# marekrams/tnac4o

Measured on AMD Instinct MI355X. Metric: PEPS-contraction ms/sweep, chimera L=2048 chi=64 (boundary-MPS sweep _setup_rhoT), lower is better.
Workload: dtype f64; 1 GPU; chimera L=2048 (Nx=Ny=16, Nc=8), synthetic couplings seed 20260004, beta=3, chi=64; one sweep = 16 rows of MPO absorb + compress_mps; one step = the sweeps of the 4 lattice rotations of one instance; parallelism=1 GPU: 4 lattice rotations of one instance interleaved on 4 HIP streams, mode=sweep

## Files before the change

include/tnpeps.h:

```cpp
#ifndef TNPEPS_H
#define TNPEPS_H
#include <stdint.h>

#ifdef __cplusplus
extern "C" {
#endif

int tn_version(void);
int tn_build_id(char* buf, int n);
int tn_stream_create_masked(const uint32_t* mask_host, int nwords, void** stream_out);
int tn_stream_destroy(void* stream);
int tn_last_error(char* buf, int n);

int tn_gemm(int64_t M, int64_t N, int64_t K, double alpha, const double* A, int64_t rsa, int64_t csa,
            const double* B, int64_t rsb, int64_t csb, double beta, double* C, int64_t rsc, int64_t csc,
            int64_t batch, int64_t bsa, int64_t bsb, int64_t bsc, void* ws, int64_t ws_bytes, void* stream);
int64_t tn_gemm_ws_bytes(int64_t M, int64_t N, int64_t K, int64_t batch);

int tn_absorb(const double* A, const double* W, double* out, int64_t Dl, int64_t pold, int64_t Dr, int64_t ba,
              int64_t po, int64_t bb, int64_t pi, int hconj, int64_t batch, int64_t bsA, int64_t bsW, int64_t bsOut,
              void* stream);

int tn_qr(double* A, int64_t rs, int64_t cs, int64_t m, int64_t n, double* Q, int64_t qrs, int64_t qcs, double* R,
          int64_t rrs, int64_t rcs, int nb, double rank_tol, int64_t* keff_host, void* ws, int64_t ws_bytes, void* stream);
int64_t tn_qr_ws_bytes(int64_t m, int64_t n, int nb);
int64_t tn_panel_orth_ws_bytes(int64_t nrows, int b);
int tn_panel_orth(const double* X, int64_t rs, int64_t cs, int64_t nrows, int b, double* Y, int64_t yrs, int64_t ycs, int method,
                  int* state9_host, double* dev_host, void* ws, int64_t ws_bytes, void* stream);
int tn_panel_stats(uint64_t* out16_host, int reset);
int tn_panel_stats_stream(uint64_t* out16_host, int reset, void* stream);
int tn_smallqr_stats(uint64_t* out4_host, int reset, void* stream);
int tn_fused_timeouts(int* count_host, void* stream);
int tn_qr_batched(double* A, int64_t rs, int64_t cs, int64_t m, int64_t n, double* Q, int64_t qrs, int64_t qcs, double* R,
                  int64_t rrs, int64_t rcs, int nb, double rank_tol, int64_t* keff_host, int64_t batch, int64_t bsA, int64_t bsQ,
                  int64_t bsR, void* ws, int64_t ws_bytes, void* stream, void* const* side_streams, int nside);

int tn_svd_trunc(const double* C, int64_t crs, int64_t ccs, int64_t k, int64_t n, int64_t Dmax, double tol, double* U,
                 int64_t urs, int64_t ucs, double* S, double* Vt, int64_t vrs, int64_t vcs, int64_t* keep_host,
                 double* discarded_host, int* sweeps_host, int* info_host, void* ws, int64_t ws_bytes, void* stream);
int tn_svdvals(const double* C, int64_t crs, int64_t ccs, int64_t k, int64_t n, double* S_host, int* sweeps_host,
               int* info_host, void* ws, int64_t ws_bytes, void* stream);
int64_t tn_svd_ws_bytes(int64_t k, int64_t n, int vectors);
int tn_svdvals_async(const double* C, int64_t crs, int64_t ccs, int64_t k, int64_t n, double* out66_dev, void* stream);
int tn_svdvals_small_batched(const int64_t* desc_dev, int64_t batch, const int64_t* desc_host, double* out66_dev, void* stream);
int tn_svd_trunc_batched(const double* C, int64_t crs, int64_t ccs, int64_t k, int64_t n, int64_t Dmax, double tol, double* U,
                         int64_t urs, int64_t ucs, double* S, double* Vt, int64_t vrs, int64_t vcs, int64_t* keep_host,
                         double* discarded_host, int* sweeps_host, int* info_host, int64_t batch, int64_t bsC, int64_t bsU,
                         int64_t bsS, int64_t bsV, void* ws, int64_t ws_bytes, void* stream);
int tn_svdvals_batched(const double* C, int64_t crs, int64_t ccs, int64_t k, int64_t n, double* S_host, int* sweeps_host,
                       int* info_host, int64_t batch, int64_t bsC, void* ws, int64_t ws_bytes, void* stream);

int tn_nfactor(const double* x, int64_t n, double* out2, void* slot8, void* stream);
int tn_normalize_pow2(double* x, int64_t n, double* out2, void* scratch, int64_t scratch_bytes, void* stream);
int tn_scale_by(double* x, int64_t n, const double* scalar_dev, void* stream);
int tn_scale_phys(double* A, int64_t Dl, int64_t p, int64_t Dr, const double* diag, int inv, void* stream);

int tn_peps_factor(const double* Es, const double* E1, const double* E4, const double* Xu, const double* Xl, const double* Xr,
                   const double* Xd, const int32_t* dmap, const int32_t* rmap, int64_t q, int64_t nl, int64_t nu, double* F,
                   void* stream);
int tn_mpo_from_factor(const double* F, const int32_t* dmap, const int32_t* rmap, int64_t q, int64_t nl, int64_t nu, int64_t pd,
                       int64_t br, double* W, void* stream);
int tn_mpo_from_factor_ops(const double* F, const int32_t* dmap, const int32_t* rmap, const double* O, int64_t nop, int64_t q, int64_t nl,
                           int64_t nu, int64_t pd, int64_t br, double* Wops, void* stream);

int tn_calc_pn(const double* T1, const double* RR, const double* F, const int32_t* dmap, const int32_t* rmap,
               const int32_t* pref, const int32_t* suf, const int32_t* lidx, const int32_t* uidx, int64_t nb,
               int64_t q, int64_t nl, int64_t nu, int64_t p, int64_t Dr, int64_t br, double* P, double* minP,
               const double* parent_log2p, double* log2p_out, void* stream);
int tn_sample_pn(const double* T1, const double* RR, const double* F, const int32_t* dmap, const int32_t* rmap, const int32_t* pref,
                 const int32_t* suf, const int32_t* lidx, const int32_t* uidx, const int32_t* perm, const int64_t* starts, int64_t ng,
// ... 124 lines not shown
```

tnac4o_amd/_lib.py:

```python
import ctypes as C
import os
import subprocess

HERE = os.path.dirname(os.path.abspath(__file__))
LIB_PATH = os.path.join(HERE, 'libtnpeps.so')
CSRC = os.path.join(HERE, 'csrc')
SOURCES = ['api.hip', 'gemm_f64.hip', 'rank_update.hip', 'small.hip', 'qr.hip', 'svd.hip', 'absorb.hip', 'misc.hip', 'beam.hip', 'prof.hip', 'cholqr.hip', 'smallqr.hip', 'fused.hip', 'peps.hip', 'env.hip', 'batch.hip', 'site.hip', 'chain.hip', 'beamsearch.hip', 'marginal.hip', 'sampler.hip', 'overlap.hip']

_i64, _f64, _int, _ptr = C.c_int64, C.c_double, C.c_int, C.c_void_p

SIGNATURES = {
    'tn_version': (_int, []),
    'tn_last_error': (_int, [C.c_char_p, _int]),
    'tn_build_id': (_int, [C.c_char_p, _int]),
    'tn_stream_create_masked': (_int, [C.POINTER(C.c_uint32), _int, C.POINTER(_ptr)]),
    'tn_stream_destroy': (_int, [_ptr]),
    'tn_gemm': (_int, [_i64, _i64, _i64, _f64, _ptr, _i64, _i64, _ptr, _i64, _i64, _f64, _ptr, _i64, _i64,
                       _i64, _i64, _i64, _i64, _ptr, _i64, _ptr]),
    'tn_gemm_ws_bytes': (_i64, [_i64, _i64, _i64, _i64]),
    'tn_absorb': (_int, [_ptr, _ptr, _ptr, _i64, _i64, _i64, _i64, _i64, _i64, _i64, _int, _i64, _i64, _i64, _i64, _ptr]),
    'tn_qr': (_int, [_ptr, _i64, _i64, _i64, _i64, _ptr, _i64, _i64, _ptr, _i64, _i64, _int, _f64, C.POINTER(_i64), _ptr, _i64,
              _ptr]),
    'tn_qr_ws_bytes': (_i64, [_i64, _i64, _int]),
    'tn_panel_orth_ws_bytes': (_i64, [_i64, _int]),
    'tn_panel_orth': (_int, [_ptr, _i64, _i64, _i64, _int, _ptr, _i64, _i64, _int, C.POINTER(_int), C.POINTER(_f64), _ptr, _i64, _ptr]),
    'tn_panel_stats': (_int, [C.POINTER(C.c_uint64), _int]),
    'tn_panel_stats_stream': (_int, [C.POINTER(C.c_uint64), _int, _ptr]),
    'tn_smallqr_stats': (_int, [C.POINTER(C.c_uint64), _int, _ptr]),
    'tn_fused_timeouts': (_int, [C.POINTER(_int), _ptr]),
    'tn_qr_batched': (_int, [_ptr, _i64, _i64, _i64, _i64, _ptr, _i64, _i64, _ptr, _i64, _i64, _int, _f64, C.POINTER(_i64), _i64, _i64, _i64,
                      _i64, _ptr, _i64, _ptr, C.POINTER(_ptr), _int]),
    'tn_svd_trunc': (_int, [_ptr, _i64, _i64, _i64, _i64, _i64, _f64, _ptr, _i64, _i64, _ptr, _ptr, _i64, _i64,
                            C.POINTER(_i64), C.POINTER(_f64), C.POINTER(_int), C.POINTER(_int), _ptr, _i64, _ptr]),
    'tn_svdvals': (_int, [_ptr, _i64, _i64, _i64, _i64, C.POINTER(_f64), C.POINTER(_int), C.POINTER(_int), _ptr, _i64,
                          _ptr]),
    'tn_svd_ws_bytes': (_i64, [_i64, _i64, _int]),
    'tn_svdvals_async': (_int, [_ptr, _i64, _i64, _i64, _i64, _ptr, _ptr]),
    'tn_svdvals_small_batched': (_int, [_ptr, _i64, _ptr, _ptr, _ptr]),
    'tn_svd_trunc_batched': (_int, [_ptr, _i64, _i64, _i64, _i64, _i64, _f64, _ptr, _i64, _i64, _ptr, _ptr, _i64, _i64, C.POINTER(_i64),
                             C.POINTER(_f64), C.POINTER(_int), C.POINTER(_int), _i64, _i64, _i64, _i64, _i64, _ptr, _i64, _ptr]),
    'tn_svdvals_batched': (_int, [_ptr, _i64, _i64, _i64, _i64, C.POINTER(_f64), C.POINTER(_int), C.POINTER(_int), _i64, _i64, _ptr, _i64,
                           _ptr]),
    'tn_nfactor': (_int, [_ptr, _i64, _ptr, _ptr, _ptr]),
    'tn_scale_by': (_int, [_ptr, _i64, _ptr, _ptr]),
    'tn_normalize_pow2': (_int, [_ptr, _i64, _ptr, _ptr, _i64, _ptr]),
    'tn_scale_phys': (_int, [_ptr, _i64, _i64, _i64, _ptr, _int, _ptr]),
    'tn_calc_pn': (_int, [_ptr] * 9 + [_i64] * 7 + [_ptr, _ptr, _ptr, _ptr, _ptr]),
    'tn_sample_pn': (_int, [_ptr] * 11 + [_i64, _ptr] + [_i64] * 6 + [_ptr, _ptr, _ptr, _ptr]),
    'tn_score_pn': (_int, [_ptr] * 11 + [_i64, _ptr] + [_i64] * 8 + [_ptr, _ptr, _ptr, _ptr, _ptr]),
    'tn_merge_groups': (_int, [_ptr] * 5 + [_i64, _f64, _ptr, _ptr, _ptr, _ptr]),
    'tn_mpo_from_factor_ops': (_int, [_ptr] * 4 + [_i64] * 6 + [_ptr, _ptr]),
    'tn_nfactor_batched': (_int, [_ptr, _i64, _i64, _ptr]),
    'tn_env_rr_batched': (_int, [_ptr] * 5 + [_i64] * 7 + [_ptr, _ptr]),
    'tn_env_rl_batched': (_int, [_ptr] * 3 + [_i64] * 3 + [_ptr, _ptr]),
    'tn_balance': (_int, [_ptr, _i64, _i64, _i64, _f64, _ptr, _ptr, _ptr]),
    'tn_peps_factor': (_int, [_ptr] * 9 + [_i64] * 3 + [_ptr, _ptr]),
    'tn_mpo_from_factor': (_int, [_ptr] * 3 + [_i64] * 5 + [_ptr, _ptr]),
    'tn_site_qr_ws_bytes': (_i64, [_int, _i64, _i64, _i64, _i64, _int]),
    'tn_site_qr': (_int, [_int, _ptr, _i64, _i64, _i64, _ptr, _i64, _ptr, _ptr, _f64, C.POINTER(_i64), _ptr, C.POINTER(_int), C.POINTER(_f64),
                   _int, C.POINTER(_i64), _ptr, _i64, _ptr]),
    'tn_gram_weights': (_int, [_ptr, _i64, _f64, _ptr, _ptr, _ptr]),
    'tn_rows_norm2': (_int, [_ptr, _i64, _i64, _ptr, _ptr]),
    'tn_gather_scale_rows': (_int, [_ptr, _i64, _i64, _ptr, _ptr, _ptr, _int, _ptr]),
    'tn_bond_deflate': (_int, [_int, _ptr, _i64, _i64, _ptr, _i64, _ptr, _ptr, C.POINTER(_i64), C.POINTER(_f64), _ptr, _i64, _ptr]),
    'tn_rar_ws_bytes': (_i64, [_i64] * 5),
    'tn_rar': (_int, [_ptr, _ptr, _ptr] + [_i64] * 5 + [_ptr, _ptr, _i64, _ptr]),
    'tn_env_mix_ws_bytes': (_i64, [_int] + [_i64] * 5),
    'tn_env_mix': (_int, [_int, _ptr, _ptr, _ptr] + [_i64] * 5 + [_ptr, _ptr, _i64, _ptr]),
    'tn_apply_truncation_ws_bytes': (_i64, [_i64] * 5),
    'tn_apply_truncation': (_int, [_ptr, _i64, _i64, _ptr, _i64, _i64, _i64, _ptr, _i64, _i64, _ptr, _i64, _i64, _ptr, _ptr, _ptr, _ptr, _ptr,
                            _i64, _ptr]),
    'tn_compress_mps_arena_bytes': (_i64, [_i64, C.POINTER(_i64), C.POINTER(_i64), _i64]),
# ... 67 lines not shown
    src_hash = source_hash()

    def one(s):
        src = os.path.join(CSRC, s)
        h = hh.copy()
        h.update(open(src, 'rb').read())
        extra = []
        if s == 'api.hip':
            extra = ['-DTN_SRC_HASH="%s"' % src_hash]
            h.update(src_hash.encode())
        obj = os.path.join(objdir, '%s.%s.o' % (s[:-4], h.hexdigest()[:16]))
        if not os.path.exists(obj):
            for old in os.listdir(objdir):
                if old.startswith(s[:-4] + '.') and old.endswith('.o'):
                    os.unlink(os.path.join(objdir, old))
            import tempfile
            fd, tmp = tempfile.mkstemp(prefix=s[:-4] + '.', suffix='.o.part', dir=objdir)
            os.close(fd)
            cmd = [hipcc] + flags + extra + ['-c', src, '-o', tmp]
            if verbose:
                print(' '.join(cmd), flush=True)
            try:
                subprocess.run(cmd, check=True)
                os.replace(tmp, obj)
            finally:
                if os.path.exists(tmp):
                    os.unlink(tmp)
        return obj

    with ThreadPoolExecutor(max_workers=int(os.environ.get('TN_BUILD_JOBS', '6'))) as ex:
        objs = list(ex.map(one, SOURCES))
    cmd = [hipcc, '--offload-arch=gfx950', '-shared', '-fPIC', '-Wl,--no-undefined'] + os.environ.get('TN_EXTRA_HIPCC_FLAGS', '').split() + ['-o', LIB_PATH] + objs
    if verbose:
        print(' '.join(cmd), flush=True)
    subprocess.run(cmd, check=True)
    return LIB_PATH


def _stale(L):
    buf = C.create_string_buffer(64)
    L.tn_build_id.restype, L.tn_build_id.argtypes = _int, [C.c_char_p, _int]
    L.tn_build_id(buf, 64)
    return buf.value.decode() != source_hash()


SHORT_CALLS = ('tn_gemm', 'tn_gemm_ws_bytes', 'tn_qr_ws_bytes', 'tn_svd_ws_bytes', 'tn_absorb', 'tn_nfactor', 'tn_scale_by',
               'tn_normalize_pow2', 'tn_scale_phys', 'tn_calc_pn', 'tn_sample_pn', 'tn_score_pn', 'tn_nfactor_batched', 'tn_env_rr_batched', 'tn_env_rl_batched',
               'tn_balance', 'tn_merge_groups', 'tn_svdvals_async', 'tn_rar', 'tn_rar_ws_bytes', 'tn_env_mix', 'tn_env_mix_ws_bytes',
               'tn_apply_truncation', 'tn_apply_truncation_ws_bytes', 'tn_site_qr_ws_bytes', 'tn_gram_weights', 'tn_argsort_desc', 'tn_weighted_sum', 'tn_rows_norm2', 'tn_gather_scale_rows', 'tn_peps_factor', 'tn_mpo_from_factor', 'tn_env3', 'tn_env3_ws_bytes',
               'tn_cluster_marginal', 'tn_cluster_marginal_ws_bytes', 'tn_cluster_bond_marginal', 'tn_cluster_bond_marginal_ws_bytes',
               'tn_mpo_from_factor_ops', 'tn_env3_stack', 'tn_env3_stack_ws_bytes', 'tn_stack_cell_law', 'tn_stack_cell_law_ws_bytes',
               'tn_last_error')
_lib = None
ABI_VERSION = 17


def lib():
    global _lib
    if _lib is None:
        if not os.path.exists(LIB_PATH):
            raise RuntimeError('libtnpeps.so not found at %s: run `python -c "import __graft_entry__ as g; g.build()"` '
                               '(the HIP library is the only backend; there is no CPU fallback)' % LIB_PATH)
        L = C.CDLL(LIB_PATH)
        L.tn_version.restype = _int
        if not hasattr(L, 'tn_build_id') or (_stale(L) and not os.environ.get('TN_ALLOW_STALE_LIB')):
            raise RuntimeError('libtnpeps.so was built from other sources than csrc/*.hip + include/tnpeps.h in this tree: '
                               'rebuild it with `python -c "import __graft_entry__ as g; g.build()"` -- a stale library can '
                               'disagree with the ctypes signatures declared here')
        if L.tn_version() != ABI_VERSION:
            raise RuntimeError('libtnpeps.so implements C-ABI version %d, this package binds version %d: rebuild the library'
                               % (L.tn_version(), ABI_VERSION))
        if os.environ.get('TN_PYDLL', '1') != '0':
            P = C.PyDLL(LIB_PATH)
            for name in SHORT_CALLS:
                setattr(L, name, getattr(P, name))
            L._pydll = P
        for name, (res, args) in SIGNATURES.items():
            fn = getattr(L, name)
            fn.restype, fn.argtypes = res, args
        _lib = L
    return _lib


class TnError(RuntimeError):
    pass


def check(rc):
    if rc != 0:
        buf = C.create_string_buffer(512)
        lib().tn_last_error(buf, 512)
        raise TnError('libtnpeps error %d: %s' % (rc, buf.value.decode(errors='replace')))
```

tnac4o_amd/csrc/api.hip:

```cpp
#include <stdarg.h>

#include "../../include/tnpeps.h"
#include "common.h"

namespace tn {

static thread_local char g_err[512] = "";

void set_error(const char* fmt, ...) {
    va_list ap;
    va_start(ap, fmt);
    vsnprintf(g_err, sizeof(g_err), fmt, ap);
    va_end(ap);
}
const char* get_error() { return g_err; }

}

using namespace tn;
#define ST ((hipStream_t)stream)

extern "C" {

int tn_version(void) { return 17; }

#ifndef TN_SRC_HASH
#define TN_SRC_HASH "unknown"
#endif
int tn_build_id(char* buf, int n) {
    const char* e = TN_SRC_HASH;
    const int len = (int)strlen(e);
    if (buf && n > 0) {
        const int c = len < n - 1 ? len : n - 1;
        memcpy(buf, e, c);
        buf[c] = 0;
    }
    return len;
}

void tn_profile_enable(unsigned mask) { prof_set_mask(mask); }
void tn_profile_reset(void) { prof_reset(); }
void tn_profile_sample(unsigned every) { prof_set_sample(every); }
int tn_profile_get(int family, uint64_t* calls_host, double* ms_host, double* flops_host, double* bytes_host) {
    TN_CHECK_ARG(family >= 0 && family < PROF_NFAM, "unknown kernel family");
    TN_CHECK_ARG(calls_host && ms_host && flops_host && bytes_host, "null output");
    prof_get(-1, family, calls_host, ms_host, flops_host, bytes_host);
    return 0;
}
int tn_profile_get_phase(int phase, int family, uint64_t* calls_host, double* ms_host, double* flops_host, double* bytes_host) {
    TN_CHECK_ARG(phase >= -1 && phase < PH_N, "unknown phase");
    TN_CHECK_ARG(family >= 0 && family < PROF_NFAM, "unknown kernel family");
    TN_CHECK_ARG(calls_host && ms_host && flops_host && bytes_host, "null output");
    prof_get(phase, family, calls_host, ms_host, flops_host, bytes_host);
    return 0;
}

int tn_stream_create_masked(const uint32_t* mask_host, int nwords, void** stream_out) {
    TN_CHECK_ARG(mask_host && nwords >= 1 && stream_out, "bad arguments");
    hipStream_t st = nullptr;
    const hipError_t e = hipExtStreamCreateWithCUMask(&st, (uint32_t)nwords, mask_host);
    if (e != hipSuccess) return hip_fail(e, "hipExtStreamCreateWithCUMask");
    fused_forms_disable(st);
    *stream_out = (void*)st;
    return 0;
}
int tn_stream_destroy(void* stream) {
    fused_stream_released((hipStream_t)stream);
    const hipError_t e = hipStreamDestroy((hipStream_t)stream);
    return e == hipSuccess ? 0 : hip_fail(e, "hipStreamDestroy");
}

int tn_last_error(char* buf, int n) {
    const char* e = get_error();
    int len = (int)strlen(e);
    if (buf && n > 0) {
        int c = len < n - 1 ? len : n - 1;
        memcpy(buf, e, c);
        buf[c] = 0;
    }
    return len;
}

int tn_gemm(int64_t M, int64_t N, int64_t K, double alpha, const double* A, int64_t rsa, int64_t csa, const double* B,
            int64_t rsb, int64_t csb, double beta, double* C, int64_t rsc, int64_t csc, int64_t batch, int64_t bsa,
            int64_t bsb, int64_t bsc, void* ws, int64_t ws_bytes, void* stream) {
    TN_CHECK_ARG(M >= 0 && N >= 0 && K >= 0 && batch >= 0, "negative dimension");
    TN_CHECK_ARG(A && B && C, "null operand");
    return gemm(ST, M, N, K, alpha, A, rsa, csa, B, rsb, csb, beta, C, rsc, csc, batch, bsa, bsb, bsc, (double*)ws, ws_bytes);
}
int64_t tn_gemm_ws_bytes(int64_t M, int64_t N, int64_t K, int64_t batch) { return gemm_ws_bytes(M, N, K, batch); }

int tn_absorb(const double* A, const double* W, double* out, int64_t Dl, int64_t pold, int64_t Dr, int64_t ba, int64_t po,
              int64_t bb, int64_t pi, int hconj, int64_t batch, int64_t bsA, int64_t bsW, int64_t bsOut, void* stream) {
    TN_CHECK_ARG(batch >= 0, "negative batch");
    TN_CHECK_ARG(batch == 0 || (A && W && out), "null operand");
    ProfPhase ph(PH_ABSORB);
    return absorb(ST, A, W, out, Dl, pold, Dr, ba, po, bb, pi, hconj, batch, bsA, bsW, bsOut);
}

int tn_qr(double* A, int64_t rs, int64_t cs, int64_t m, int64_t n, double* Q, int64_t qrs, int64_t qcs, double* R, int64_t rrs,
          int64_t rcs, int nb, double rank_tol, int64_t* keff_host, void* ws, int64_t ws_bytes, void* stream) {
    TN_CHECK_ARG(A && Q && R && ws, "null operand");
    TN_CHECK_ARG(rank_tol >= 0.0 && rank_tol < 1.0, "rank_tol out of range");
    ProfPhase ph(PH_QR);
    prof_note_qr(m, n, 1);
    return qr_factor(ST, A, rs, cs, m, n, Q, qrs, qcs, R, rrs, rcs, nb, ws, ws_bytes, rank_tol, keff_host);
}
int64_t tn_qr_ws_bytes(int64_t m, int64_t n, int nb) { return qr_ws_bytes(m, n, nb); }

int tn_smallqr_stats(uint64_t* out4_host, int reset, void* stream) {
    TN_CHECK_ARG(out4_host, "null output");
    unsigned long long o[4];
    const int rc = smallqr_stats(ST, o, reset);
    for (int i = 0; i < 4; ++i) out4_host[i] = o[i];
    return rc;
}
int tn_fused_timeouts(int* count_host, void* stream) {
    TN_CHECK_ARG(count_host, "null output");
    return fused_timeouts(ST, count_host);
}

int64_t tn_panel_orth_ws_bytes(int64_t nrows, int b) { return cholqr_ws_bytes(nrows, b); }
int tn_panel_orth(const double* X, int64_t rs, int64_t cs, int64_t nrows, int b, double* Y, int64_t yrs, int64_t ycs, int method,
                  int* state9_host, double* dev_host, void* ws, int64_t ws_bytes, void* stream) {
    TN_CHECK_ARG(X && Y && ws, "null operand");
    TN_CHECK_ARG(method == 0, "method must be 0 (Cholesky-QR)");
    TN_CHECK_ARG(b >= 1 && b <= 32, "panel width must be <= 32");
    TN_CHECK_ARG(ws_bytes >= tn_panel_orth_ws_bytes(nrows, b), "workspace too small");
    ProfPhase ph(PH_QR);
    int rc = cholqr_reset(ST, ws);
    if (rc) return rc;
    int fbase = 0;
    if ((rc = cholqr_orthonormalize(ST, X, rs, cs, Y, yrs, ycs, nrows, b, ws, ws_bytes, 0x5DEECE66DULL, &fbase))) return rc;
    if (fused_check_needed() && !fused_check_deferred()) {
        int gave_up = 0;
        if ((rc = fused_timeouts(ST, &gave_up))) return rc;
        if (gave_up > 0) {
            if ((rc = cholqr_reset(ST, ws))) return rc;
            fbase = 0;
            if ((rc = cholqr_orthonormalize(ST, X, rs, cs, Y, yrs, ycs, nrows, b, ws, ws_bytes, 0x5DEECE66DULL, &fbase))) return rc;
        }
    }
    if (state9_host && dev_host) return cholqr_debug_state(ST, ws, state9_host, dev_host);
// ... 206 lines not shown
```

tnac4o_amd/csrc/chain.hip:

```cpp
#include <math.h>
#include <stdlib.h>

#include <cmath>

#include <algorithm>
#include <chrono>
#include <map>
#include <memory>
#include <mutex>
#include <vector>

#include "common.h"

namespace tn {

__global__ __launch_bounds__(256) void permute4_kernel(const double* __restrict__ in, int64_t s0, int64_t s1, int64_t s2, int64_t s3, int64_t n0,
                                                       int64_t n1, int64_t n2, int64_t n3, double* __restrict__ out) {
    const int64_t tot = n0 * n1 * n2 * n3;
    for (int64_t e = (int64_t)blockIdx.x * 256 + threadIdx.x; e < tot; e += (int64_t)gridDim.x * 256) {
        const int64_t i3 = e % n3, r = e / n3, i2 = r % n2, r2 = r / n2, i1 = r2 % n1, i0 = r2 / n1;
        out[e] = in[i0 * s0 + i1 * s1 + i2 * s2 + i3 * s3];
    }
}
static int permute4(hipStream_t st, const double* in, int64_t s0, int64_t s1, int64_t s2, int64_t s3, int64_t n0, int64_t n1, int64_t n2, int64_t n3,
// ... 548 lines not shown
        if ((pass_side == 0 ? site.c : site.a) != k) { set_error("tn_compress_mps: centre matrix does not fit its site"); return -1; }
        M2 Cn;
        T3 Sn;
        if (pass_side == 0) { CH(new_m2(k, n, Cn, "deflated centre")); CH(new_t3(site.a, site.b, k, Sn, "deflated site")); }
        else { CH(new_m2(n, k, Cn, "deflated centre")); CH(new_t3(k, site.b, site.c, Sn, "deflated site")); }
        void* w = nullptr;
        CH(scratch(3, 8192, w));
        int64_t kk = k;
        double d2 = 0.0;
        CH(bond_deflate(st, pass_side, C.p, k, n, site.p, m, Cn.p, Sn.p, &kk, &d2, w, 8192));
        if (kk == k) return 0;
        if (pass_side == 0) { Cn.r = kk; Sn.c = kk; ar.shrink((char*)Cn.p, kk * n * 8); ar.shrink((char*)Sn.p, m * kk * 8); }
        else { Cn.c = kk; Sn.a = kk; ar.shrink((char*)Cn.p, n * kk * 8); ar.shrink((char*)Sn.p, kk * m * 8); }
        site = Sn;
        C = Cn;
        D[pC] = kk;
        discarded[pC] = std::max(discarded[pC], std::sqrt(d2));
        bonds_deflated += k - kk;
        return 0;
    }
    int64_t bonds_deflated = 0;
    std::vector<M2> pass_C;
    int canonise_left(bool compress, int64_t Dmax, double tol) {
        pass_side = 0;
        CH(ones11(C));
        pC = 0;
        pass_C.assign((size_t)L + 1, M2());
        for (int64_t n = 0; n < L; ++n) {
            const double rank_tol = (compress && 0 < n + 1 && n + 1 < L) ? CH_RANK_TOL : 0.0;
            const M2 Cm = C;
            PassMark tm(st);
            if (compress) tm.substart();
            CH(site_left(n, &Cm, rank_tol));
            if (compress) { tm.trlap(pass_id, 0); trmark = &tm; CH(truncateC(Dmax, tol)); trmark = nullptr; }
            if (compress && intermediate_pass) pass_C[pC] = C;
        }
        return 0;
    }
    int canonise_right(bool compress, int64_t Dmax, double tol) {
        pass_side = 1;
        CH(ones11(C));
        pC = L;
        for (int64_t n = L - 1; n >= 0; --n) {
            const double rank_tol = (compress && 0 < n && n < L) ? CH_RANK_TOL : 0.0;
            const M2 Cm = C;
            PassMark tm(st);
            if (compress) tm.substart();
            CH(site_right(n, &Cm, rank_tol));
            if (compress) { tm.trlap(pass_id, 0); trmark = &tm; CH(truncateC(Dmax, tol)); trmark = nullptr; }
        }
        return 0;
    }

    int gram_step_structured(M2& G, int64_t n) {
        const int64_t* fd = &facdims[7 * n];
        const int64_t Dl = fd[0], ps = fd[1], Dr = fd[2], ba = fd[3], po = fd[4], bb = fd[5], pi = fd[6];
        const double* Af = facA[n];
        const double* W = facW[n];
        const int64_t wl = po * bb * pi, wr = pi;
        const int64_t wsd = hconj ? bb * pi : 1, wtd = hconj ? 1 : bb * pi;
        const int64_t pt = hconj ? pi : po;
        const int64_t na = Dl * ba;
        Ref gpb; double* Gp = nullptr;
        CH(new_block(na * ba * Dl, gpb, Gp, "Gram (permuted)"));
        if (hconj) CH(permute4(st, G.p, ba * na, na, 1, ba, Dl, ba, ba, Dl, Gp));
        else CH(permute4(st, G.p, na, Dl * na, Dl, 1, Dl, ba, ba, Dl, Gp));
        Ref t1b; double* T1 = nullptr;
        CH(new_block(na * ba * ps * Dr, t1b, T1, "Gram step T1"));
        CH(mm(na * ba, ps * Dr, Dl, Gp, Dl, 1, Af, ps * Dr, 1, T1, ps * Dr, 1));
        gpb.reset();
        Ref wxb; double* Wx = nullptr;
        CH(new_block(pt * bb * ba * ps, wxb, Wx, "Wx"));
        CH(permute4(st, W, wtd, wr, wl, wsd, pt, bb, ba, ps, Wx));
        Ref t2b; double* T2 = nullptr;
        CH(new_block(na * pt * bb * Dr, t2b, T2, "Gram step T2"));
        CH(bmm(na, pt * bb, Dr, ba * ps, Wx, ba * ps, 1, 0, T1, Dr, 1, ba * ps * Dr, T2, Dr, 1, pt * bb * Dr));
        t1b.reset();
        Ref wyb; double* Wy = nullptr;
        CH(new_block(ps * bb * ba * pt, wyb, Wy, "Wy"));
        CH(permute4(st, W, wsd, wr, wl, wtd, ps, bb, ba, pt, Wy));
        Ref ub; double* U = nullptr;
        CH(new_block(Dl * ps * bb * bb * Dr, ub, U, "Gram step U"));
        CH(bmm(Dl, ps * bb, bb * Dr, ba * pt, Wy, ba * pt, 1, 0, T2, bb * Dr, 1, ba * pt * bb * Dr, U, bb * Dr, 1, ps * bb * bb * Dr));
        t2b.reset();
        Ref ob; double* O = nullptr;
        CH(new_block(Dr * bb * bb * Dr, ob, O, "Gram step O"));
        CH(mm(Dr, bb * bb * Dr, Dl * ps, Af, 1, Dr, U, bb * bb * Dr, 1, O, bb * bb * Dr, 1));
        ub.reset();
        M2 Gn;
        CH(new_m2(Dr * bb, Dr * bb, Gn, "Gram matrix"));
        if (hconj) CH(permute4(st, O, bb * bb * Dr, bb * Dr, 1, Dr, Dr, bb, Dr, bb, Gn.p));
        else CH(permute4(st, O, bb * Dr, bb * bb * Dr, Dr, 1, bb, Dr, bb, Dr, Gn.p));
        G = Gn;
        return 0;
    }
    int ensure_absorbed(int64_t n) {
        if (A[n].p) return 0;
        if (facA.empty() || !facA[n]) { set_error("tn_compress_mps: site %lld has neither a tensor nor its factors", (long long)n); return -1; }
        const int64_t* fd = &facdims[7 * n];
        T3 t;
        CH(new_t3(A[n].a, A[n].b, A[n].c, t, "absorbed site"));
        {
            ProfPhase ph(PH_ABSORB);
            CH(absorb(st, facA[n], facW[n], t.p, fd[0], fd[1], fd[2], fd[3], fd[4], fd[5], fd[6], hconj, 1, 0, 0, 0));
        }
        A[n] = t;
        return 0;
    }
    int attach_through_factors(int64_t n, const M2& Cm, double* Am) {
        const int64_t* fd = &facdims[7 * n];
        const int64_t Dl = fd[0], ps = fd[1], Dr = fd[2], ba = fd[3], po = fd[4], bb = fd[5], pi = fd[6], r = Cm.c;
        const int64_t pt = hconj ? pi : po;
        if (Cm.r != Dr * bb || (hconj ? po : pi) != ps) { set_error("tn_compress_mps: centre matrix does not fit the factors of site %lld", (long long)n); return -1; }
        Ref tb; double* T = nullptr;
        CH(new_block(Dl * ps * bb * r, tb, T, "attach through the factors: T"));
        if (hconj) CH(mm(Dl * ps, bb * r, Dr, facA[n], Dr, 1, Cm.p, bb * r, 1, T, bb * r, 1));
        else CH(bmm(bb, Dl * ps, r, Dr, facA[n], Dr, 1, 0, Cm.p, r, 1, Dr * r, T, bb * r, 1, r));
        Ref wb; double* Wq = nullptr;
        CH(new_block(ba * pt * ps * bb, wb, Wq, "attach through the factors: W"));
        if (hconj) CH(permute4(st, facW[n], po * bb * pi, 1, bb * pi, pi, ba, pt, ps, bb, Wq));
        else CH(permute4(st, facW[n], po * bb * pi, bb * pi, 1, pi, ba, pt, ps, bb, Wq));
        if (hconj) return bmm(Dl, ba * pt, r, ps * bb, Wq, ps * bb, 1, 0, T, r, 1, ps * bb * r, Am, r, 1, ba * pt * r);
        Ref mb; double* Mt = nullptr;
        CH(new_block(Dl * ba * pt * r, mb, Mt, "attach through the factors: M (MPS-major)"));
        CH(bmm(Dl, ba * pt, r, ps * bb, Wq, ps * bb, 1, 0, T, r, 1, ps * bb * r, Mt, r, 1, ba * pt * r));
        return permute4(st, Mt, pt * r, ba * pt * r, r, 1, ba, Dl, pt, r, Am);
    }
    int canonise_right_weighted(bool& accepted) {
        struct Wt { Ref blk; double* d2 = nullptr; double* st65 = nullptr; bool on = false; };
        std::vector<Wt> wts(L + 1);
        std::vector<double*> gfac(L + 1, nullptr);
        M2 G;
        PassMark sm(st);
        sm.substart();
        CH(ones11(G));
        for (int64_t n = 0; n < L; ++n) {
            const int64_t Dl = A[n].a, p = A[n].b, Dr = A[n].c;
            const bool structured = !facA.empty() && facA[n] != nullptr && Dl >= CH_PASS1_MIN_BOND && G.r == Dl;
            if (structured) CH(gram_step_structured(G, n));
            else {
                CH(ensure_absorbed(n));
                Ref xb; double* X = nullptr;
                CH(new_block(Dl * p * Dr, xb, X, "Gram step X"));
                CH(mm(Dl, p * Dr, Dl, G.p, Dl, 1, A[n].p, p * Dr, 1, X, p * Dr, 1));
                M2 Gn;
                CH(new_m2(Dr, Dr, Gn, "Gram matrix"));
                CH(mm(Dr, Dr, Dl * p, A[n].p, 1, Dr, X, Dr, 1, Gn.p, Dr, 1));
                G = Gn;
            }
            gfac[n + 1] = next_nf();
            CH(normalize(G.p, G.r * G.c, gfac[n + 1]));
            if (n + 1 < L && Dr >= CH_PASS1_MIN_BOND) {
                Wt& w = wts[n + 1];
                double* q = nullptr;
                CH(new_block(Dr + 65, w.blk, q, "bond weights"));
                w.d2 = q; w.st65 = q + Dr; w.on = true;
                CH(gram_weights(st, G.p, Dr, CH_PASS1_FLOOR, w.d2, w.st65));
            }
        }
        sm.sublap(0);
        std::vector<int64_t> used;
        for (int64_t n = 0; n < L; ++n) if (wts[n].on) used.push_back(n);
        if (used.empty()) {
            CH(canonise_right(false, 0, 0.0));
            reveal_error_bound = 0.0;
            accepted = true;
// ... 513 lines not shown
```

tnac4o_amd/csrc/common.h:

```cpp
#pragma once
#include <hip/hip_runtime.h>
#include <stdint.h>
#include <stdio.h>
#include <stdlib.h>
#include <string.h>

namespace tn {

void set_error(const char* fmt, ...);
const char* get_error();

inline int hip_fail(hipError_t e, const char* what) {
    set_error("%s: %s", what, hipGetErrorString(e));
    return (int)e > 0 ? (int)e : 1;
}

#define TN_CHECK_ARG(cond, msg)                \
    do {                                       \
        if (!(cond)) {                         \
            tn::set_error("%s: %s", __func__, msg); \
            return -1;                         \
        }                                      \
    } while (0)

// ... 63 lines not shown
void prof_note_qr(int64_t m, int64_t n, int64_t batch);
void prof_note_svd(int64_t k, int64_t n, int sweeps);
void prof_note_svdvals(int64_t k, int64_t n);
int prof_phase(int phase);
struct ProfPhase {
    int prev;
    explicit ProfPhase(int ph) : prev(prof_phase(ph)) {}
    ~ProfPhase() { prof_phase(prev); }
};
#define TN_PROF_LAUNCH(st, fam, launch) do { prof_begin(st, fam); launch; prof_end(st, fam, 0.0, 0.0); } while (0)
void prof_set_mask(unsigned mask);
void prof_set_sample(unsigned n);
void prof_reset();
void prof_get(int phase, int fam, uint64_t* calls, double* ms, double* flops, double* bytes);

struct Mat {
    double* p;
    int64_t rs, cs;
};
static inline Mat mat(double* p, int64_t rs, int64_t cs) { return Mat{p, rs, cs}; }
static inline Mat sub(Mat a, int64_t i, int64_t j) { return Mat{a.p + i * a.rs + j * a.cs, a.rs, a.cs}; }
static inline Mat tr(Mat a) { return Mat{a.p, a.cs, a.rs}; }

int gemm(hipStream_t st, int64_t M, int64_t N, int64_t K, double alpha, const double* A, int64_t rsa, int64_t csa,
         const double* B, int64_t rsb, int64_t csb, double beta, double* C, int64_t rsc, int64_t csc,
         int64_t batch = 1, int64_t bsa = 0, int64_t bsb = 0, int64_t bsc = 0, double* ws = nullptr,
         int64_t ws_bytes = 0);
int64_t gemm_ws_bytes(int64_t M, int64_t N, int64_t K, int64_t batch);
struct GemmExtra {
    const int* pairs = nullptr;
    const int* skip = nullptr;
    int pw = 0, mapA = 0, mapB = 0, mapC = 0;
    int force_splitk = 0;
    bool raw_partials = false;
    int* splitk_used = nullptr;
};
int gemm_forced_split(int64_t K, int s, int64_t* kchunk);
int gemm_ex(hipStream_t st, int64_t M, int64_t N, int64_t K, double alpha, const double* A, int64_t rsa, int64_t csa,
            const double* B, int64_t rsb, int64_t csb, double beta, double* C, int64_t rsc, int64_t csc, int64_t batch,
            int64_t bsa, int64_t bsb, int64_t bsc, double* ws, int64_t ws_bytes, const GemmExtra* x);

static inline int gemm(hipStream_t st, int64_t M, int64_t N, int64_t K, double alpha, Mat A, Mat B, double beta, Mat C,
                       double* ws = nullptr, int64_t ws_bytes = 0) {
    return gemm(st, M, N, K, alpha, A.p, A.rs, A.cs, B.p, B.rs, B.cs, beta, C.p, C.rs, C.cs, 1, 0, 0, 0, ws, ws_bytes);
}
int gemm_prof_family(int64_t M, int64_t N, int64_t K, int64_t rsc, int64_t csc);

int rank_update(hipStream_t st, int64_t m, int64_t n, int b, const double* W, int64_t wrs, int64_t wcs, const double* X, int64_t xrs,
                int64_t xcs, double* C, int64_t rsc, int64_t csc, const int* active);
static inline int rank_update(hipStream_t st, int64_t m, int64_t n, int b, Mat W, Mat X, Mat C, const int* active = nullptr) {
    return rank_update(st, m, n, b, W.p, W.rs, W.cs, X.p, X.rs, X.cs, C.p, C.rs, C.cs, active);
}

constexpr int NBMAX = 64;

int gram_partial(hipStream_t st, const double* X, int64_t vs, int64_t es, int64_t L, int nvec, int w, const int* pairs,
                 int ngroups, int nchunk, double* part);
int gram_nchunk(int64_t L);

int eig_small(hipStream_t st, const double* part, int nchunk, int nvec, int ngroups, int mode, int max_sweeps,
              double dead_thresh, double* out, int* dead, int* nrot, double* maxoff, double relevant2 = 0.0, int allow_fast = 1);

int rows_times_small(hipStream_t st, double* X, int64_t rs, int64_t cs, int64_t nrows, int b, const double* S);

struct SvdRoundsJob {
    double* X; int64_t pitch, L; int nvp, w;
    const int* pairs; int ng, nr, nchunk;
    double* part; int64_t part_bytes; double* Js; int* nrot; double* maxoff;
    double relevant2, last_tol; int inner_first, inner_later;
    double* norms;
};
int svd_rounds_fused(hipStream_t st, const SvdRoundsJob& j);
int small_t_times_vecs(hipStream_t st, const double* S, double* X, int64_t vs, int64_t es, int64_t L, int nvec, int w,
                       const int* pairs, int ngroups, const int* nrot);


int qr_factor(hipStream_t st, double* A, int64_t rs, int64_t cs, int64_t m, int64_t n, double* Q, int64_t qrs, int64_t qcs, double* R,
              int64_t rrs, int64_t rcs, int nb, void* ws, int64_t ws_bytes, double rank_tol, int64_t* keff_host,
              double* dropped2_host = nullptr, int frob_exit = 0, int64_t* pivot_perm_host = nullptr, double* nf_out2 = nullptr,
              int* nf_done = nullptr);
int64_t qr_ws_bytes(int64_t m, int64_t n, int nb);


constexpr int CQ_MAXPASS = 4;
constexpr double CQ_THETA = 1e-10;
constexpr double CQ_DONE = 5e-15;
constexpr double CQ_LAST = 1e-8;
int64_t cholqr_ws_bytes(int64_t nrows, int b);
int cholqr_reset(hipStream_t st, void* ws);
int cholqr_begin(hipStream_t st, void* ws, void** state_out);
void cholqr_end_ok(hipStream_t st);
int cholqr_orthonormalize(hipStream_t st, const double* X, int64_t irs, int64_t ics, double* Y, int64_t rs, int64_t cs, int64_t nrows,
                          int b, void* ws, int64_t ws_bytes, uint64_t seed, int* fused_base, void* state = nullptr);
int cholqr_panel(hipStream_t st, const double* X, int64_t irs, int64_t ics, double* Y, int64_t rs, int64_t cs, int64_t nrows, int b, void* ws,
                 int64_t ws_bytes, uint64_t seed, int reconstruct, double* Tp, double* W, int64_t wrs, int64_t wcs, double* Wq, int* fused_base,
                 void* state = nullptr, const int* active = nullptr);
int cholqr_debug_state(hipStream_t st, const void* ws, int* ints9, double* dev_hist);
int cholqr_stats(unsigned long long* out16, int reset, hipStream_t st_or_null, int all_streams);
bool smallqr_fits(int64_t m, int64_t n);
int64_t smallqr_ws_bytes(int64_t m, int64_t n);
int smallqr_factor(hipStream_t st, const double* A, int64_t rs, int64_t cs, int64_t m, int64_t n, double* Q, int64_t qrs, int64_t qcs, double* R,
                   int64_t rrs, int64_t rcs, double* nf_out2, void* ws, int64_t ws_bytes);

constexpr int CQ_FUSED_MAXBLK = 32;
constexpr unsigned CQ_SPIN_LIMIT = 1u << 22;
constexpr int CHOLQR_SLOTS = 64;
// ... 110 lines not shown
```

Baseline: 364.9 ms/sweep.

## Fuse the two chained factor GEMMs into one MFMA kernel with an LDS intermediate

Adds a factor_products kernel that computes the first product (P·X) per z and column chunk into LDS, then multiplies the W factor against it in the same workgroup with f64 MFMA. It is used in the Gram step and in attach-through-factors of compress_mps when the shapes fit. This removes the intermediate T1/T buffer round trip through global memory and one launch per step. The cost is occupancy, since each workgroup holds a 128KB LDS slab, plus possible redundant reads of W across z blocks.

New measurement: 358.0 ms/sweep (median of 6 runs). 1.02x faster.

```diff
diff --git a/include/tnpeps.h b/include/tnpeps.h
--- a/include/tnpeps.h
+++ b/include/tnpeps.h
@@ -16,6 +16,13 @@
             const double* B, int64_t rsb, int64_t csb, double beta, double* C, int64_t rsc, int64_t csc,
             int64_t batch, int64_t bsa, int64_t bsb, int64_t bsc, void* ws, int64_t ws_bytes, void* stream);
 int64_t tn_gemm_ws_bytes(int64_t M, int64_t N, int64_t K, int64_t batch);
+
+int tn_factor_products_eligible(int64_t Z, int64_t I, int64_t J, int64_t K1, int64_t N, int64_t M, int first_batched);
+int64_t tn_factor_products_ws_bytes(int64_t Z, int64_t I, int64_t J, int64_t K1, int64_t N, int first_batched);
+int tn_factor_products(int64_t Z, int64_t I, int64_t J, int64_t K1, int64_t N, int64_t Mhi, int64_t Mlo, const double* P, int64_t pz,
+                       int64_t pi, int64_t pk, const double* X, int64_t xk, int64_t xj, int64_t xn, const double* W, int64_t wm,
+                       int64_t wq, double* Out, int64_t oz, int64_t ohi, int64_t olo, int64_t on, int first_batched, void* ws,
+                       int64_t ws_bytes, void* stream);
 
 int tn_absorb(const double* A, const double* W, double* out, int64_t Dl, int64_t pold, int64_t Dr, int64_t ba,
               int64_t po, int64_t bb, int64_t pi, int hconj, int64_t batch, int64_t bsA, int64_t bsW, int64_t bsOut,
diff --git a/tnac4o_amd/_lib.py b/tnac4o_amd/_lib.py
--- a/tnac4o_amd/_lib.py
+++ b/tnac4o_amd/_lib.py
@@ -5,7 +5,7 @@
 HERE = os.path.dirname(os.path.abspath(__file__))
 LIB_PATH = os.path.join(HERE, 'libtnpeps.so')
 CSRC = os.path.join(HERE, 'csrc')
-SOURCES = ['api.hip', 'gemm_f64.hip', 'rank_update.hip', 'small.hip', 'qr.hip', 'svd.hip', 'absorb.hip', 'misc.hip', 'beam.hip', 'prof.hip', 'cholqr.hip', 'smallqr.hip', 'fused.hip', 'peps.hip', 'env.hip', 'batch.hip', 'site.hip', 'chain.hip', 'beamsearch.hip', 'marginal.hip', 'sampler.hip', 'overlap.hip']
+SOURCES = ['api.hip', 'gemm_f64.hip', 'rank_update.hip', 'factor_products.hip', 'small.hip', 'qr.hip', 'svd.hip', 'absorb.hip', 'misc.hip', 'beam.hip', 'prof.hip', 'cholqr.hip', 'smallqr.hip', 'fused.hip', 'peps.hip', 'env.hip', 'batch.hip', 'site.hip', 'chain.hip', 'beamsearch.hip', 'marginal.hip', 'sampler.hip', 'overlap.hip']
 
 _i64, _f64, _int, _ptr = C.c_int64, C.c_double, C.c_int, C.c_void_p
 
@@ -18,6 +18,10 @@
     'tn_gemm': (_int, [_i64, _i64, _i64, _f64, _ptr, _i64, _i64, _ptr, _i64, _i64, _f64, _ptr, _i64, _i64,
                        _i64, _i64, _i64, _i64, _ptr, _i64, _ptr]),
     'tn_gemm_ws_bytes': (_i64, [_i64, _i64, _i64, _i64]),
+    'tn_factor_products_eligible': (_int, [_i64] * 6 + [_int]),
+    'tn_factor_products_ws_bytes': (_i64, [_i64] * 5 + [_int]),
+    'tn_factor_products': (_int, [_i64] * 7 + [_ptr, _i64, _i64, _i64, _ptr, _i64, _i64, _i64, _ptr, _i64, _i64, _ptr, _i64, _i64, _i64, _i64,
+                                  _int, _ptr, _i64, _ptr]),
     'tn_absorb': (_int, [_ptr, _ptr, _ptr, _i64, _i64, _i64, _i64, _i64, _i64, _i64, _int, _i64, _i64, _i64, _i64, _ptr]),
     'tn_qr': (_int, [_ptr, _i64, _i64, _i64, _i64, _ptr, _i64, _i64, _ptr, _i64, _i64, _int, _f64, C.POINTER(_i64), _ptr, _i64,
               _ptr]),
@@ -191,7 +195,7 @@
                'tn_mpo_from_factor_ops', 'tn_env3_stack', 'tn_env3_stack_ws_bytes', 'tn_stack_cell_law', 'tn_stack_cell_law_ws_bytes',
                'tn_last_error')
 _lib = None
-ABI_VERSION = 17
+ABI_VERSION = 18
 
 
 def lib():
diff --git a/tnac4o_amd/csrc/api.hip b/tnac4o_amd/csrc/api.hip
--- a/tnac4o_amd/csrc/api.hip
+++ b/tnac4o_amd/csrc/api.hip
@@ -22,7 +22,7 @@
 
 extern "C" {
 
-int tn_version(void) { return 17; }
+int tn_version(void) { return 18; }
 
 #ifndef TN_SRC_HASH
 #define TN_SRC_HASH "unknown"
@@ -89,6 +89,46 @@
     return gemm(ST, M, N, K, alpha, A, rsa, csa, B, rsb, csb, beta, C, rsc, csc, batch, bsa, bsb, bsc, (double*)ws, ws_bytes);
 }
 int64_t tn_gemm_ws_bytes(int64_t M, int64_t N, int64_t K, int64_t batch) { return gemm_ws_bytes(M, N, K, batch); }
+
+int tn_factor_products_eligible(int64_t Z, int64_t I, int64_t J, int64_t K1, int64_t N, int64_t M, int first_batched) {
+    return factor_products_fits(Z, I, J, K1, N, M) && (first_batched || gemm_ws_bytes(Z * I, J * N, K1, 1) == 0) ? 1 : 0;
+}
+static int64_t factor_products_layout(char* base, int64_t Z, int64_t I, int64_t J, int64_t K1, int64_t N, int first_batched, double** S,
+                                      double** gw, int64_t* gw_bytes) {
+    WsCarve c{base};
+    *gw_bytes = first_batched ? 0 : gemm_ws_bytes(Z * I, J * N, K1, 1);
+    *S = c.take<double>(Z * I * J * N * 8);
+    *gw = c.take<double>(*gw_bytes);
+    return c.total();
+}
+int64_t tn_factor_products_ws_bytes(int64_t Z, int64_t I, int64_t J, int64_t K1, int64_t N, int first_batched) {
+    double* S; double* gw; int64_t gb;
+    return factor_products_layout(nullptr, Z, I, J, K1, N, first_batched, &S, &gw, &gb);
+}
+int tn_factor_products(int64_t Z, int64_t I, int64_t J, int64_t K1, int64_t N, int64_t Mhi, int64_t Mlo, const double* P, int64_t pz,
+                       int64_t pi, int64_t pk, const double* X, int64_t xk, int64_t xj, int64_t xn, const double* W, int64_t wm,
+                       int64_t wq, double* Out, int64_t oz, int64_t ohi, int64_t olo, int64_t on, int first_batched, void* ws,
+                       int64_t ws_bytes, void* stream) {
+    TN_CHECK_ARG(Z >= 1 && I >= 1 && J >= 1 && K1 >= 1 && N >= 1 && Mhi >= 1 && Mlo >= 1, "non-positive dimension");
+    TN_CHECK_ARG(P && X && W && Out, "null operand");
+    TN_CHECK_ARG((Z == 1 || pz == I * pi) && (first_batched || J == 1 || xj == N * xn), "the first product needs pz = I pi, and unbatched xj = N xn");
+    if (factor_products_on() && tn_factor_products_eligible(Z, I, J, K1, N, Mhi * Mlo, first_batched)) {
+        FactorProducts f;
+        f.Z = Z; f.I = I; f.J = J; f.K1 = K1; f.N = N; f.Mhi = Mhi; f.Mlo = Mlo;
+        f.P = P; f.pz = pz; f.pi = pi; f.pk = pk; f.X = X; f.xk = xk; f.xj = xj; f.xn = xn; f.W = W; f.wm = wm; f.wq = wq;
+        f.Out = Out; f.oz = oz; f.ohi = ohi; f.olo = olo; f.on = on;
+        return factor_products(ST, f);
+    }
+    double* S; double* gw; int64_t gb;
+    const int64_t need = factor_products_layout((char*)ws, Z, I, J, K1, N, first_batched, &S, &gw, &gb);
+    TN_CHECK_ARG(ws && ws_bytes >= need, "workspace too small (tn_factor_products_ws_bytes)");
+    int rc;
+    if (first_batched) rc = gemm(ST, Z * I, N, K1, 1.0, P, pi, pk, X, xk, xn, 0.0, S, J * N, 1, J, 0, xj, N, nullptr, 0);
+    else rc = gemm(ST, Z * I, J * N, K1, 1.0, P, pi, pk, X, xk, xn, 0.0, S, J * N, 1, 1, 0, 0, 0, gw, gb);
+    for (int64_t h = 0; h < Mhi && rc == 0; ++h)
+        rc = gemm(ST, Mlo, N, I * J, 1.0, W + h * Mlo * wm, wm, wq, S, N, 1, 0.0, Out + h * ohi, olo, on, Z, 0, I * J * N, oz, nullptr, 0);
+    return rc;
+}
 
 int tn_absorb(const double* A, const double* W, double* out, int64_t Dl, int64_t pold, int64_t Dr, int64_t ba, int64_t po,
               int64_t bb, int64_t pi, int hconj, int64_t batch, int64_t bsA, int64_t bsW, int64_t bsOut, void* stream) {
diff --git a/tnac4o_amd/csrc/chain.hip b/tnac4o_amd/csrc/chain.hip
--- a/tnac4o_amd/csrc/chain.hip
+++ b/tnac4o_amd/csrc/chain.hip
@@ -624,6 +624,9 @@
         return 0;
     }
 
+    static bool factor_pair_fused(int64_t Z, int64_t I, int64_t J, int64_t K1, int64_t N, int64_t M, int64_t M1, int64_t N1) {
+        return factor_products_on() && factor_products_fits(Z, I, J, K1, N, M) && (M1 == 0 || gemm_ws_bytes(M1, N1, K1, 1) == 0);
+    }
     int gram_step_structured(M2& G, int64_t n) {
         const int64_t* fd = &facdims[7 * n];
         const int64_t Dl = fd[0], ps = fd[1], Dr = fd[2], ba = fd[3], po = fd[4], bb = fd[5], pi = fd[6];
@@ -637,17 +640,30 @@
         CH(new_block(na * ba * Dl, gpb, Gp, "Gram (permuted)"));
         if (hconj) CH(permute4(st, G.p, ba * na, na, 1, ba, Dl, ba, ba, Dl, Gp));
         else CH(permute4(st, G.p, na, Dl * na, Dl, 1, Dl, ba, ba, Dl, Gp));
-        Ref t1b; double* T1 = nullptr;
-        CH(new_block(na * ba * ps * Dr, t1b, T1, "Gram step T1"));
-        CH(mm(na * ba, ps * Dr, Dl, Gp, Dl, 1, Af, ps * Dr, 1, T1, ps * Dr, 1));
-        gpb.reset();
         Ref wxb; double* Wx = nullptr;
-        CH(new_block(pt * bb * ba * ps, wxb, Wx, "Wx"));
-        CH(permute4(st, W, wtd, wr, wl, wsd, pt, bb, ba, ps, Wx));
         Ref t2b; double* T2 = nullptr;
-        CH(new_block(na * pt * bb * Dr, t2b, T2, "Gram step T2"));
-        CH(bmm(na, pt * bb, Dr, ba * ps, Wx, ba * ps, 1, 0, T1, Dr, 1, ba * ps * Dr, T2, Dr, 1, pt * bb * Dr));
-        t1b.reset();
+        if (factor_pair_fused(na, ba, ps, Dl, Dr, pt * bb, na * ba, ps * Dr)) {
+            CH(new_block(pt * bb * ba * ps, wxb, Wx, "Wx"));
+            CH(permute4(st, W, wl, wsd, wtd, wr, ba, ps, pt, bb, Wx));
+            CH(new_block(na * pt * bb * Dr, t2b, T2, "Gram step T2"));
+            FactorProducts f;
+            f.Z = na; f.I = ba; f.J = ps; f.K1 = Dl; f.N = Dr; f.Mhi = 1; f.Mlo = pt * bb;
+            f.P = Gp; f.pz = ba * Dl; f.pi = Dl; f.pk = 1;
+            f.X = Af; f.xk = ps * Dr; f.xj = Dr; f.xn = 1;
+            f.W = Wx; f.wm = 1; f.wq = pt * bb;
+            f.Out = T2; f.oz = pt * bb * Dr; f.ohi = 0; f.olo = Dr; f.on = 1;
+            CH(factor_products(st, f));
+            gpb.reset();
+        } else {
+            Ref t1b; double* T1 = nullptr;
+            CH(new_block(na * ba * ps * Dr, t1b, T1, "Gram step T1"));
+            CH(mm(na * ba, ps * Dr, Dl, Gp, Dl, 1, Af, ps * Dr, 1, T1, ps * Dr, 1));
+            gpb.reset();
+            CH(new_block(pt * bb * ba * ps, wxb, Wx, "Wx"));
+            CH(permute4(st, W, wtd, wr, wl, wsd, pt, bb, ba, ps, Wx));
+            CH(new_block(na * pt * bb * Dr, t2b, T2, "Gram step T2"));
+            CH(bmm(na, pt * bb, Dr, ba * ps, Wx, ba * ps, 1, 0, T1, Dr, 1, ba * ps * Dr, T2, Dr, 1, pt * bb * Dr));
+        }
         Ref wyb; double* Wy = nullptr;
         CH(new_block(ps * bb * ba * pt, wyb, Wy, "Wy"));
         CH(permute4(st, W, wsd, wr, wl, wtd, ps, bb, ba, pt, Wy));
@@ -684,6 +700,19 @@
         const int64_t Dl = fd[0], ps = fd[1], Dr = fd[2], ba = fd[3], po = fd[4], bb = fd[5], pi = fd[6], r = Cm.c;
         const int64_t pt = hconj ? pi : po;
         if (Cm.r != Dr * bb || (hconj ? po : pi) != ps) { set_error("tn_compress_mps: centre matrix does not fit the factors of site %lld", (long long)n); return -1; }
+        if (factor_pair_fused(Dl, ps, bb, Dr, r, ba * pt, hconj ? Dl * ps : 0, bb * r)) {
+            Ref wb; double* Wq = nullptr;
+            CH(new_block(ba * pt * ps * bb, wb, Wq, "attach through the factors: W"));
+            if (hconj) CH(permute4(st, facW[n], bb * pi, pi, po * bb * pi, 1, ps, bb, ba, pt, Wq));
+            else CH(permute4(st, facW[n], 1, pi, po * bb * pi, bb * pi, ps, bb, ba, pt, Wq));
+            FactorProducts f;
+            f.Z = Dl; f.I = ps; f.J = bb; f.K1 = Dr; f.N = r; f.Mhi = ba; f.Mlo = pt;
+            f.P = facA[n]; f.pz = ps * Dr; f.pi = Dr; f.pk = 1;
+            f.X = Cm.p; f.xk = hconj ? bb * r : r; f.xj = hconj ? r : Dr * r; f.xn = 1;
+            f.W = Wq; f.wm = 1; f.wq = ba * pt;
+            f.Out = Am; f.oz = hconj ? ba * pt * r : pt * r; f.ohi = hconj ? pt * r : Dl * pt * r; f.olo = r; f.on = 1;
+            return factor_products(st, f);
+        }
         Ref tb; double* T = nullptr;
         CH(new_block(Dl * ps * bb * r, tb, T, "attach through the factors: T"));
         if (hconj) CH(mm(Dl * ps, bb * r, Dr, facA[n], Dr, 1, Cm.p, bb * r, 1, T, bb * r, 1));
diff --git a/tnac4o_amd/csrc/common.h b/tnac4o_amd/csrc/common.h
--- a/tnac4o_amd/csrc/common.h
+++ b/tnac4o_amd/csrc/common.h
@@ -139,6 +139,17 @@
     return rank_update(st, m, n, b, W.p, W.rs, W.cs, X.p, X.rs, X.cs, C.p, C.rs, C.cs, active);
 }
 
+struct FactorProducts {
+    int64_t Z, I, J, K1, N, Mhi, Mlo;
+    const double* P; int64_t pz, pi, pk;
+    const double* X; int64_t xk, xj, xn;
+    const double* W; int64_t wm, wq;
+    double* Out; int64_t oz, ohi, olo, on;
+};
+bool factor_products_fits(int64_t Z, int64_t I, int64_t J, int64_t K1, int64_t N, int64_t M);
+inline bool factor_products_on() { return env_flag_on("TN_FACTOR_FUSED"); }
+int factor_products(hipStream_t st, const FactorProducts& f);
+
 constexpr int NBMAX = 64;
 
 int gram_partial(hipStream_t st, const double* X, int64_t vs, int64_t es, int64_t L, int nvec, int w, const int* pairs,
diff --git a/tnac4o_amd/csrc/factor_products.hip b/tnac4o_amd/csrc/factor_products.hip
--- /dev/null
+++ b/tnac4o_amd/csrc/factor_products.hip
@@ -0,0 +1,200 @@
+#include "common.h"
+
+namespace tn {
+
+namespace {
+
+typedef double d4 __attribute__((ext_vector_type(4)));
+
+constexpr int FP_NC = 64;
+constexpr int FP_QMAX = 256;
+constexpr int FP_IMAX = 16;
+constexpr int FP_K1MAX = 64;
+constexpr int FP_THREADS = 512, FP_WAVES = FP_THREADS / 64;
+constexpr int FP_SLAB = 32 * FP_WAVES;
+
+struct FacP {
+    const double* P;
+    const double* X;
+    const double* W;
+    double* Out;
+    int Z, I, J, K1, N, M, Mlo, chunks;
+    int64_t pz, pi, pk, xk, xj, xn, wm, wq, oz, ohi, olo, on;
+};
+
+__device__ __forceinline__ int fp_sidx(int q, int c) { return q * FP_NC + (c ^ ((q & 1) << 4)); }
+
+__device__ __forceinline__ double fp_keep(double v, bool keep) {
+    long long m = keep ? -1ll : 0ll;
+    asm volatile("" : "+v"(m));
+    return __longlong_as_double(__double_as_longlong(v) & m);
+}
+
+template <int KS>
+__device__ __forceinline__ void fp_stage1(const FacP& g, double* S, const int z, const int n0, const int nb, const int wave, const int lr, const int lk) {
+    constexpr int KG = 4 * KS;
+    double p[KG];
+    {
+        const double* Pz = g.P + (int64_t)z * g.pz + (int64_t)min(lr, g.I - 1) * g.pi;
+#pragma unroll
+        for (int kk = 0; kk < KG; ++kk) {
+            const int k = kk * 4 + lk;
+            const double v = Pz[(int64_t)min(k, g.K1 - 1) * g.pk];
+            p[kk] = fp_keep(v, lr < g.I && k < g.K1);
+        }
+    }
+    const int units = g.J * nb;
+    auto load = [&](double (&b)[KG], const int u) {
+        const int uc = min(u, units - 1), j = uc / nb, cb = uc - j * nb, n = n0 + cb * 16 + lr;
+        const double* Xp = g.X + (int64_t)j * g.xj + (int64_t)min(n, g.N - 1) * g.xn;
+#pragma unroll
+        for (int kk = 0; kk < KG; ++kk) {
+            const int k = kk * 4 + lk;
+            const double v = Xp[(int64_t)min(k, g.K1 - 1) * g.xk];
+            b[kk] = fp_keep(v, n < g.N && k < g.K1);
+        }
+    };
+    auto multiply = [&](const double (&b)[KG], const int u) {
+        if (u >= units) return;
+        d4 acc = d4{0.0, 0.0, 0.0, 0.0};
+#pragma unroll
+        for (int kk = 0; kk < KG; ++kk) acc = __builtin_amdgcn_mfma_f64_16x16x4f64(p[kk], b[kk], acc, 0, 0, 0);
+        const int j = u / nb, cb = u - j * nb;
+#pragma unroll
+        for (int r = 0; r < 4; ++r) {
+            const int i = lk + 4 * r;
+            if (i < g.I) S[fp_sidx(i * g.J + j, cb * 16 + lr)] = acc[r];
+        }
+    };
+    double b0[KG], b1[KG];
+    load(b0, wave);
+    for (int u = wave; u < units; u += 2 * FP_WAVES) {
+        load(b1, u + FP_WAVES);
+        multiply(b0, u);
+        load(b0, u + 2 * FP_WAVES);
+        multiply(b1, u + FP_WAVES);
+    }
+}
+
+template <int TN>
+__device__ __forceinline__ void fp_stage2(const FacP& g, const double* S, const int z, const int n0, const int Q, const int m0, const int lr, const int lk) {
+    const double* Wr[2];
+    bool rv[2];
+#pragma unroll
+    for (int i = 0; i < 2; ++i) {
+        const int m = m0 + i * 16 + lr;
+        rv[i] = m < g.M;
+        Wr[i] = g.W + (int64_t)min(m, g.M - 1) * g.wm;
+    }
+    auto load = [&](double (&a)[4][2], const int qs) {
+#pragma unroll
+        for (int kk = 0; kk < 4; ++kk) {
+            const int q = qs + kk * 4 + lk;
+            const int64_t off = (int64_t)min(q, Q - 1) * g.wq;
+#pragma unroll
+            for (int i = 0; i < 2; ++i) {
+                const double v = Wr[i][off];
+                a[kk][i] = fp_keep(v, rv[i] && q < Q);
+            }
+        }
+    };
+    d4 acc[2][TN];
+#pragma unroll
+    for (int i = 0; i < 2; ++i)
+#pragma unroll
+        for (int j = 0; j < TN; ++j) acc[i][j] = d4{0.0, 0.0, 0.0, 0.0};
+    double ac[4][2], an[4][2];
+    load(ac, 0);
+    for (int qs = 0; qs < Q; qs += 16) {
+        load(an, qs + 16);
+#pragma unroll
+        for (int kk = 0; kk < 4; ++kk) {
+            const int q = qs + kk * 4 + lk;
+            double b[TN];
+#pragma unroll
+            for (int j = 0; j < TN; ++j) b[j] = S[fp_sidx(q, j * 16 + lr)];
+#pragma unroll
+            for (int i = 0; i < 2; ++i)
+#pragma unroll
+                for (int j = 0; j < TN; ++j) acc[i][j] = __builtin_amdgcn_mfma_f64_16x16x4f64(ac[kk][i], b[j], acc[i][j], 0, 0, 0);
+        }
+#pragma unroll
+        for (int kk = 0; kk < 4; ++kk)
+#pragma unroll
+            for (int i = 0; i < 2; ++i) ac[kk][i] = an[kk][i];
+    }
+    double* Oz = g.Out + (int64_t)z * g.oz;
+#pragma unroll
+    for (int i = 0; i < 2; ++i)
+#pragma unroll
+        for (int r = 0; r < 4; ++r) {
+            const int m = m0 + i * 16 + lk + 4 * r;
+            if (m >= g.M) continue;
+            const int mh = m / g.Mlo, ml = m - mh * g.Mlo;
+            double* o = Oz + (int64_t)mh * g.ohi + (int64_t)ml * g.olo;
+#pragma unroll
+            for (int j = 0; j < TN; ++j) {
+                const int n = n0 + j * 16 + lr;
+                if (n < g.N) o[(int64_t)n * g.on] = acc[i][j][r];
+            }
+        }
+}
+
+template <int KS>
+__global__ __launch_bounds__(FP_THREADS) void factor_products_kernel(FacP g) {
+    __shared__ double S[FP_QMAX * FP_NC];
+    const int tid = threadIdx.x, lane = tid & 63, wave = __builtin_amdgcn_readfirstlane(tid >> 6);
+    const int lr = lane & 15, lk = lane >> 4;
+    int bid = blockIdx.x;
+    {
+        const int nwg = gridDim.x, q = nwg / 8, r = nwg % 8, xcd = bid % 8, loc = bid / 8;
+        bid = (xcd < r ? xcd * (q + 1) : r * (q + 1) + (xcd - r) * q) + loc;
+    }
+    const int z = bid / g.chunks, n0 = (bid - z * g.chunks) * FP_NC;
+    const int nb = (min(FP_NC, g.N - n0) + 15) >> 4;
+    const int Q = g.I * g.J, Qpad = (Q + 15) & ~15;
+    for (int e = Q * FP_NC + tid; e < Qpad * FP_NC; e += FP_THREADS) S[e] = 0.0;
+    fp_stage1<KS>(g, S, z, n0, nb, wave, lr, lk);
+    __syncthreads();
+    for (int mt = 0; mt < g.M; mt += FP_SLAB) {
+        const int m0 = mt + wave * 32;
+        if (m0 >= g.M) break;
+        if (nb == 4) fp_stage2<4>(g, S, z, n0, Q, m0, lr, lk);
+        else if (nb == 3) fp_stage2<3>(g, S, z, n0, Q, m0, lr, lk);
+        else if (nb == 2) fp_stage2<2>(g, S, z, n0, Q, m0, lr, lk);
+        else fp_stage2<1>(g, S, z, n0, Q, m0, lr, lk);
+    }
+}
+
+}
+
+bool factor_products_fits(int64_t Z, int64_t I, int64_t J, int64_t K1, int64_t N, int64_t M) {
+    if (Z < 1 || I < 1 || J < 1 || K1 < 1 || N < 1 || M < 1) return false;
+    if (I > FP_IMAX || I * J > FP_QMAX || K1 > FP_K1MAX) return false;
+    return M < ((int64_t)1 << 30) && N < ((int64_t)1 << 30) && Z * cdiv(N, FP_NC) < ((int64_t)1 << 31);
+}
+
+int factor_products(hipStream_t st, const FactorProducts& f) {
+    TN_CHECK_ARG(factor_products_fits(f.Z, f.I, f.J, f.K1, f.N, f.Mhi * f.Mlo) && f.Mhi >= 1 && f.Mlo >= 1, "shape outside the kernel's limits");
+    FacP g;
+    g.P = f.P; g.X = f.X; g.W = f.W; g.Out = f.Out;
+    g.Z = (int)f.Z; g.I = (int)f.I; g.J = (int)f.J; g.K1 = (int)f.K1; g.N = (int)f.N; g.M = (int)(f.Mhi * f.Mlo); g.Mlo = (int)f.Mlo;
+    g.chunks = (int)cdiv(f.N, FP_NC);
+    g.pz = f.pz; g.pi = f.pi; g.pk = f.pk; g.xk = f.xk; g.xj = f.xj; g.xn = f.xn; g.wm = f.wm; g.wq = f.wq;
+    g.oz = f.oz; g.ohi = f.ohi; g.olo = f.olo; g.on = f.on;
+    const dim3 grid((unsigned)(f.Z * g.chunks));
+    const double Q = (double)(f.I * f.J), M = (double)g.M;
+    prof_begin(st, PROF_GEMM_64x64);
+    switch (cdiv(f.K1, 16)) {
+        case 1: hipLaunchKernelGGL((factor_products_kernel<1>), grid, dim3(FP_THREADS), 0, st, g); break;
+        case 2: hipLaunchKernelGGL((factor_products_kernel<2>), grid, dim3(FP_THREADS), 0, st, g); break;
+        case 3: hipLaunchKernelGGL((factor_products_kernel<3>), grid, dim3(FP_THREADS), 0, st, g); break;
+        default: hipLaunchKernelGGL((factor_products_kernel<4>), grid, dim3(FP_THREADS), 0, st, g); break;
+    }
+    TN_CHECK_LAUNCH("factor_products_kernel");
+    prof_end(st, PROF_GEMM_64x64, 2.0 * f.Z * f.N * Q * ((double)f.K1 + M),
+             8.0 * ((double)f.Z * f.I * f.K1 + (double)f.K1 * f.J * f.N + M * Q + (double)f.Z * M * f.N));
+    return 0;
+}
+
+}
```
